# vislearn/esac

Measured on NVIDIA H100. Metric: pose hypotheses scored/sec (640x480, 256 hyp x E experts), higher is better.
Workload: dtype f32 (scoring) / f64 (P3P, refinement)

## Files before the change

__graft_entry__.py:

```python
from __future__ import annotations

import sys
from pathlib import Path

ROOT = Path(__file__).resolve().parent
if str(ROOT) not in sys.path:
    sys.path.insert(0, str(ROOT))


def build() -> None:
    from esac_b200.build import build_library
    from oracle.build import build_oracle
    from oracle.build_ref import build_ref
    lib = build_library()
    assert lib.exists()
    build_oracle()
    build_ref()
    import esac_b200.api as api
    api.load_library()
    import esac


def smoke() -> None:
    import numpy as np
    import torch
    assert torch.cuda.is_available(), "smoke() needs cuda:0"
    import esac
    import esac_b200.api as api
    from esac_b200.synth import make_scene, pose_error
    from oracle import esac_oracle as O

    sc = make_scene(E=2, H=30, W=40, M=32, sub=8, seed=1)
    api.context(0).set_option("fixed_seed", 1)
    api.set_seed(42, 0)
    out = np.zeros((4, 4), np.float32)
    e = esac.forward(sc.coords, sc.assign, out, *sc.params)
    ref = np.zeros((4, 4), np.float32)
    re_, tr = O.forward(sc.coords, sc.assign, ref, *sc.params, seed=42, trace=True)
    hy = api.last_hypotheses(0)
    ds = float(np.abs(hy["scores"] - np.array(tr.scores)).max())
    rot, trans = pose_error(out, ref)
    assert ds < 1e-4, f"score parity {ds}"
    assert e == re_ and rot < 1e-3 and trans < 1e-5, (e, re_, rot, trans)
    api.set_seed(42, 0)
    coords = torch.from_numpy(sc.coords).cuda()
    grads = torch.zeros_like(coords)
    loss = esac.backward(coords, grads, torch.from_numpy(sc.assign).cuda(), torch.from_numpy(sc.gt_pose), 1.0, 100.0,
                         100.0, *sc.params)
    g_ref = np.zeros_like(sc.coords)
    l_ref = O.backward(sc.coords, g_ref, sc.assign, sc.gt_pose, 1.0, 100.0, 100.0, *sc.params, seed=42)
    dg = float(np.abs(grads.cpu().numpy() - g_ref).max() / max(1e-12, np.abs(g_ref).max()))
    assert abs(loss - l_ref) < 1e-6 * max(1.0, abs(l_ref)), (loss, l_ref)
    assert dg < 1e-3, f"gradient parity {dg}"
    print(f"smoke ok: expert {e}, score diff {ds:.2e}, pose diff {rot:.2e} deg / {trans:.2e} m, "
          f"loss {loss:.6f} (oracle {l_ref:.6f}), grad rel diff {dg:.2e}, stats {api.last_stats(0)}")


if __name__ == "__main__":
    build()
    if len(sys.argv) > 1 and sys.argv[1] == "smoke":
        smoke()
```

esac_b200/api.py:

```python
from __future__ import annotations

import ctypes as C
import os
from pathlib import Path

import numpy as np

_HERE = Path(__file__).resolve().parent
LIB_PATH = _HERE / "libesac_b200.so"


class Stats(C.Structure):
    _fields_ = [("M", C.c_int), ("winner", C.c_int), ("n_contrib", C.c_int), ("refine_rounds", C.c_int),
                ("entropy", C.c_double), ("expected_loss", C.c_double),
                ("ms_h2d", C.c_float), ("ms_prep", C.c_float), ("ms_sample", C.c_float), ("ms_score", C.c_float),
                ("ms_select", C.c_float), ("ms_refine", C.c_float), ("ms_backward", C.c_float), ("ms_total", C.c_float),
                ("score_launches", C.c_int), ("kernel_launches", C.c_int),
                ("score_ppt", C.c_int), ("score_grid", C.c_int), ("refine_group", C.c_int)]

    def as_dict(self):
        return {k: getattr(self, k) for k, _ in self._fields_}


_lib = None
# ... 23 lines not shown
    cam = [i32, i32, f32, f32, f32, f32, f32, f32, f32, i32]
    lib.esacb200_forward.argtypes = [vp, vp, i32, i32, i32, vp, i64, i32, vp] + cam + [C.POINTER(i32)]
    lib.esacb200_backward.argtypes = [vp, vp, vp, i32, i32, i32, vp, i64, i32, vp, f32, f32, f32] + cam + [C.POINTER(f64)]
    lib.esacb200_forward_batch.argtypes = [vp, i32, vp, i32, i32, i32, vp, i64, i32, vp] + cam + [vp]
    lib.esacb200_forward_batch.restype = i32
    lib.esacb200_forward_pack.argtypes = [vp, vp, i32, i32, i32, vp, i64, i32, i32] + cam + [i32, vp]
    lib.esacb200_forward_pack.restype = i32
    lib.esacb200_nccl_unique_id.argtypes = [vp]
    lib.esacb200_nccl_unique_id.restype = i32
    lib.esacb200_comm_init.argtypes = [vp, i32, i32, vp]
    lib.esacb200_comm_init.restype = i32
    lib.esacb200_comm_destroy.argtypes = [vp]
    lib.esacb200_comm_destroy.restype = i32
    lib.esacb200_forward_sharded.argtypes = [vp, vp, i32, i32, i32, vp, i64, i32, i32, vp] + cam + [i32, C.POINTER(i32)]
    lib.esacb200_forward_sharded.restype = i32
    lib.esacb200_backward_sharded_nccl.argtypes = [vp, vp, vp, i32, i32, i32, vp, i64, i32, vp, f32, f32, f32] + cam + [i32, C.POINTER(f64)]
    lib.esacb200_backward_sharded_nccl.restype = i32
    lib.esacb200_backward_batch.argtypes = ([vp, i32, vp, vp, i32, i32, i32, vp, i64, i32, vp, f32, f32, f32, vp, vp] + cam[2:] +
                                             [vp])
    lib.esacb200_backward_batch.restype = i32
    lib.esacb200_assign_hypotheses.argtypes = [vp, i32, i32, i32, vp, i32, i32, C.c_uint64, vp, vp]
    lib.esacb200_assign_hypotheses.restype = i32
    lib.esacb200_reproj_loss.argtypes = [vp, i32, vp, vp, i32, i32, vp, vp, vp, f32, f32, f32, i32, f32, f32, f32, vp]
    lib.esacb200_reproj_loss.restype = i32
    lib.esacb200_backward_sharded.argtypes = ([vp, vp, vp, i32, i32, i32, vp, i64, i32, vp, f32, f32, f32] + cam +
                                               [EXCHANGE_FN, vp, C.POINTER(f64)])
    lib.esacb200_backward_sharded.restype = i32
    lib.esacb200_score_poses.argtypes = [vp, vp, i32, i32, i32, vp, i64, i32, vp] + cam + [vp]
    lib.esacb200_refine_poses.argtypes = [vp, vp, i32, i32, i32, vp, i64, i32, vp, i32, i32, f32, f32, f32, f32, f32, i32, vp, vp]
    lib.esacb200_get_refine_profile.argtypes = [vp, vp]
    lib.esacb200_get_refine_profile.restype = i32
    lib.esacb200_get_sample_trace.argtypes = [vp, vp]
    lib.esacb200_get_sample_trace.restype = i32
    lib.esacb200_get_sample_profile.argtypes = [vp, vp]
    lib.esacb200_get_sample_profile.restype = i32
    lib.esacb200_get_stats.argtypes = [vp, C.POINTER(Stats)]
    lib.esacb200_get_hypotheses.argtypes = [vp, vp, vp, vp, vp, vp, vp, vp]
    lib.esacb200_device_info.argtypes = [vp, C.POINTER(i32), C.c_char_p, i32]
    lib.esacb200_copy_last_scores.argtypes = [vp, vp, i32]
    lib.esacb200_copy_last_scores.restype = i32
    for name in ("set_stream", "set_seed", "set_option", "inject_cells", "forward", "backward", "score_poses",
                 "refine_poses", "get_stats", "get_hypotheses", "device_info"):
        getattr(lib, "esacb200_" + name).restype = i32
    lib.esacb200_host_rodrigues.argtypes = [vp, vp, vp]
    lib.esacb200_host_rodrigues.restype = None
    lib.esacb200_host_rodrigues_inv.argtypes = [vp, vp]
    lib.esacb200_host_rodrigues_inv.restype = None
    lib.esacb200_host_p3p_all.argtypes = [vp, vp, vp, vp]
    lib.esacb200_host_p3p_all.restype = i32
    lib.esacb200_host_p3p_pose.argtypes = [vp, vp, f32, f32, f32, f32, vp, C.POINTER(i32)]
    lib.esacb200_host_p3p_pose.restype = i32
    lib.esacb200_host_try.argtypes = [vp, vp, f32, f32, f32, f32, f32, C.POINTER(i32), C.POINTER(i32)]
    lib.esacb200_host_try.restype = None
    lib.esacb200_host_try_verdict.argtypes = [vp, vp, f32, f32, f32, f32, C.POINTER(i32), vp]
    lib.esacb200_host_try_verdict.restype = None
    lib.esacb200_host_project.argtypes = [vp, f32, f32, f32, vp, vp, vp, vp]
    lib.esacb200_host_project.restype = None
    lib.esacb200_host_loss.argtypes = [vp, vp, f64, f64, f64]
    lib.esacb200_host_loss.restype = f64
    lib.esacb200_host_dloss.argtypes = [vp, vp, f64, f64, f64, vp]
    lib.esacb200_host_dloss.restype = None
    lib.esacb200_host_pose2trans.argtypes = [vp, vp]
    lib.esacb200_host_pose2trans.restype = None
    lib.esacb200_host_trans2pose.argtypes = [vp, vp]
    lib.esacb200_host_trans2pose.restype = None
    lib.esacb200_host_dprojectdobj.argtypes = [vp, vp, vp, f32, f32, f32, f32, vp]
    lib.esacb200_host_dprojectdobj.restype = None
    lib.esacb200_host_pinv6.argtypes = [vp, vp]
    lib.esacb200_host_pinv6.restype = None
    lib.esacb200_host_draw_cells.argtypes = [C.c_uint64, C.c_uint32, C.c_uint32, i32, i32, vp]
    lib.esacb200_host_draw_cells.restype = None
    _lib = lib
    return lib


class Context:
    def __init__(self, device: int = 0):
        self.lib = load_library()
        h = C.c_void_p()
        rc = self.lib.esacb200_create(int(device), C.byref(h))
        if rc != 0:
            raise RuntimeError(f"esac_b200: cannot create a context on CUDA device {device} (status {rc}); "
                               "this implementation has no CPU path")
        self.handle = h
        self.device = int(device)
        self.comm_world, self.comm_rank = 1, 0

    def close(self):
        if getattr(self, "handle", None):
            self.lib.esacb200_destroy(self.handle)
            self.handle = None

    def __del__(self):
        try:
            self.close()
        except Exception:
            pass

    def check(self, rc: int):
        if rc != 0:
            msg = self.lib.esacb200_last_error(self.handle)
            raise RuntimeError(f"esac_b200 (status {rc}): {msg.decode() if msg else ''}")

    def set_seed(self, seed: int):
        self.check(self.lib.esacb200_set_seed(self.handle, C.c_uint64(seed & ((1 << 64) - 1))))

# ... 531 lines not shown
```

esac_b200/csrc/capi.cu:

```cuda
#include <cuda_runtime.h>
#include <dlfcn.h>
#include <stdarg.h>
#include <stdio.h>
#include <stdlib.h>
#include <string.h>

#include <exception>
#include <new>
#include <vector>
#include <thread>
#include <chrono>

#include "../../include/esac_b200.h"
#include "../../include/esac_b200_testhooks.h"
#include "esac_internal.h"
#include "esac_p3p_fast.cuh"
#include "esac_rng.cuh"

using namespace esacb200;

namespace {

struct DevBuf {
    void* p = nullptr;
    size_t cap = 0;
    cudaError_t ensure(size_t bytes) {
        if (bytes <= cap) return cudaSuccess;
        if (p) cudaFree(p);
        p = nullptr;
        cap = 0;
        size_t want = bytes + bytes / 4 + 256;
        cudaError_t e = cudaMalloc(&p, want);
        if (e == cudaSuccess) cap = want;
        return e;
    }
    void release() {
        if (p) cudaFree(p);
        p = nullptr;
        cap = 0;
    }
    template <class T>
    T* as() const { return (T*)p; }
};

enum { EV_START = 0, EV_H2D, EV_PREP, EV_SAMPLE, EV_FOLD, EV_SCORE, EV_SELECT, EV_REFINE, EV_BWD, EV_END, EV_COUNT };

}

struct esacb200_ctx {
    int device = 0;
    int sm_count = 0;
    char dev_name[128] = {0};
    cudaStream_t own_stream = nullptr;
    cudaStream_t copy_stream = nullptr;
    cudaStream_t aux_stream = nullptr;
    cudaStream_t aux_more[2] = {nullptr, nullptr};
    cudaEvent_t ev_fork = nullptr, ev_join = nullptr, ev_join_more[2] = {nullptr, nullptr};
    int sample_groups = 2;
    int upload_split = 1;
    cudaEvent_t ev_copied[2] = {nullptr, nullptr}, ev_consumed[2] = {nullptr, nullptr};
    cudaStream_t stream = nullptr;
    uint64_t seed = 1305;
    uint64_t calls = 0;
    int max_tries = 1000000;
    int max_ref_steps = 100;
    int fixed_seed = 0;
    int refine_group_opt = 0;
    int* h_flags = nullptr;
    int h_flags_cap = 0;
    int refine_pretest = 1;
    int refine_compact = 1;
    int refine_profile = 0;
    int refine_jobs_per_group = 3;
    int sample_prefilter = 1;
    int sample_span0 = 256;
    float sample_window = 1.25f;
    int sample_waves = 6;
    float sample_tail_boost = 1.f;
    int sample_trace = 0;
    int smp_groups_last = 0;
    int smp_Mg_last = 0;
    int hyp_offset = 0, hyp_stride = 1;
    int score_ppt_opt = 0, score_hc_opt = 0;
    int refine_coresident = 0;
    char err[512] = {0};
    DevBuf coords, grads, assign64, assign32, counts, offsets, perm, slot_of, chunks, scalars, centres, poses, poses_ref,
        cells, tries, posepk, part, scores, probs, stats, contrib, masks, rounds, scratch, barrier, out17, inject,
        losses, red, hypgrad, job_of, gt, smp_int, smp_surv, smp_trace, clist, eflags, coords4, coords_alt, assign64_alt, out_batch, prof;
    float* h_out = nullptr;
    double* h_dbl = nullptr;
    int inj_M = 0, inj_T = 0;
    cudaEvent_t ev[EV_COUNT] = {nullptr};
    bool ev_used[EV_COUNT] = {false};
    esacb200_stats st;
    int last_M = 0;
    bool last_backward = false;
    int batch_workers = 8;
    void* nccl_comm = nullptr;
    int comm_world = 1, comm_rank = 0;
    DevBuf gathered, grads_work;
    std::vector<esacb200_ctx*> workers;
};

namespace {

struct DeviceGuard {
    int prev = -1;
    explicit DeviceGuard(int device) {
        if (cudaGetDevice(&prev) != cudaSuccess) { cudaGetLastError(); prev = -1; }
        if (prev != device) cudaSetDevice(device);
    }
    ~DeviceGuard() {
        if (prev >= 0) cudaSetDevice(prev);
    }
    DeviceGuard(const DeviceGuard&) = delete;
    DeviceGuard& operator=(const DeviceGuard&) = delete;
};

struct NcclApi {
    typedef struct { char internal[128]; } UniqueId;
    int (*GetUniqueId)(UniqueId*) = nullptr;
    int (*CommInitRank)(void**, int, UniqueId, int) = nullptr;
    int (*CommDestroy)(void*) = nullptr;
    int (*AllGather)(const void*, void*, size_t, int, void*, cudaStream_t) = nullptr;
    int (*AllReduce)(const void*, void*, size_t, int, int, void*, cudaStream_t) = nullptr;
    const char* (*GetErrorString)(int) = nullptr;
    bool ok = false;
};
constexpr int kNcclFloat32 = 7;
// ... 1356 lines not shown
    if (probs) CK(cudaMemcpy(probs, ctx->probs.p, (size_t)M * 8, cudaMemcpyDeviceToHost));
    if (refined6) CK(cudaMemcpy(refined6, ctx->poses_ref.p, (size_t)M * sizeof(Pose), cudaMemcpyDeviceToHost));
    if (losses) {
        if (!ctx->last_backward) return fail(ctx, ESACB200_ERR_ARG, "losses exist only after backward");
        CK(cudaMemcpy(losses, ctx->losses.p, (size_t)M * 8, cudaMemcpyDeviceToHost));
    }
    return ESACB200_OK;
} ESAC_ABI_CATCH(ctx)

void esacb200_host_rodrigues(const double r[3], double R[9], double J[27]) { rodrigues_v2m(r, R, J); }
void esacb200_host_rodrigues_inv(const double R[9], double r[3]) { rodrigues_m2v(R, r); }

int esacb200_host_p3p_all(const double* y9, const double* x9, double* Rs36, double* ts12) {
    double y[3][3], x[3][3], Rs[4][9], ts[4][3];
    for (int i = 0; i < 3; ++i)
        for (int c = 0; c < 3; ++c) { y[i][c] = y9[i * 3 + c]; x[i][c] = x9[i * 3 + c]; }
    int n = p3p_solve(y, x, Rs, ts);
    for (int s = 0; s < n; ++s) {
        for (int c = 0; c < 9; ++c) Rs36[s * 9 + c] = Rs[s][c];
        for (int c = 0; c < 3; ++c) ts12[s * 3 + c] = ts[s][c];
    }
    return n;
}

int esacb200_host_p3p_pose(const float* obj12, const float* img8, float f, float ppx, float ppy, float tau, double* pose6,
                           int* gate) {
    float obj[4][3], img[4][2];
    for (int i = 0; i < 4; ++i) {
        for (int c = 0; c < 3; ++c) obj[i][c] = obj12[i * 3 + c];
        for (int c = 0; c < 2; ++c) img[i][c] = img8[i * 2 + c];
    }
    Pose p;
    bool ok = p3p_pose(obj, img, (double)f, (double)ppx, (double)ppy, p);
    if (gate) *gate = 0;
    if (!ok) { for (int i = 0; i < 6; ++i) pose6[i] = 0; return 0; }
    for (int i = 0; i < 3; ++i) { pose6[i] = p.r[i]; pose6[3 + i] = p.t[i]; }
    if (gate) *gate = minimal_set_gate(obj, img, p, (double)f, (double)ppx, (double)ppy, tau) ? 1 : 0;
    return 1;
}

void esacb200_host_try(const float* obj12, const float* img8, float f, float ppx, float ppy, float tau, float margin,
                       int* may_pass, int* accept) {
    float obj[4][3], img[4][2];
    for (int i = 0; i < 4; ++i) {
        for (int c = 0; c < 3; ++c) obj[i][c] = obj12[i * 3 + c];
        for (int c = 0; c < 2; ++c) img[i][c] = img8[i * 2 + c];
    }
    *may_pass = p3p_may_pass_fast(obj, img, f, ppx, ppy, tau, margin) ? 1 : 0;
    Pose p;
    bool ok = p3p_pose(obj, img, (double)f, (double)ppx, (double)ppy, p);
    *accept = (ok && minimal_set_gate(obj, img, p, (double)f, (double)ppx, (double)ppy, tau)) ? 1 : 0;
}

void esacb200_host_try_verdict(const float* obj12, const float* img8, float f, float ppx, float ppy, float tau, int* accept,
                               double* pose6) {
    float obj[4][3], img[4][2];
    for (int i = 0; i < 4; ++i) {
        for (int c = 0; c < 3; ++c) obj[i][c] = obj12[i * 3 + c];
        for (int c = 0; c < 2; ++c) img[i][c] = img8[i * 2 + c];
    }
    Pose p;
    const bool ok = p3p_pose(obj, img, (double)f, (double)ppx, (double)ppy, p, 1.25 * (double)tau + 1.);
    *accept = (ok && minimal_set_gate(obj, img, p, (double)f, (double)ppx, (double)ppy, tau)) ? 1 : 0;
    if (pose6 && ok)
        for (int i = 0; i < 3; ++i) { pose6[i] = p.r[i]; pose6[3 + i] = p.t[i]; }
}

void esacb200_host_project(const double pose6[6], float f, float ppx, float ppy, const float X[3], float uv_f[2],
                           double uv[2], double J12[12]) {
    double R[9], dRdr[27];
    rodrigues_v2m(pose6, R, dRdr);
    project_point_f(R, pose6 + 3, (double)f, (double)ppx, (double)ppy, X[0], X[1], X[2], uv_f[0], uv_f[1]);
    double Ju[6], Jv[6];
    project_point_jac(R, pose6 + 3, dRdr, (double)f, (double)ppx, (double)ppy, (double)X[0], (double)X[1], (double)X[2], uv[0],
                      uv[1], Ju, Jv);
    for (int i = 0; i < 6; ++i) { J12[i] = Ju[i]; J12[6 + i] = Jv[i]; }
}

double esacb200_host_loss(const double* T1, const double* T2, double wRot, double wTrans, double cut) {
    return pose_loss(T1, T2, wRot, wTrans, cut);
}

void esacb200_host_dloss(const double est6[6], const double gt6[6], double wRot, double wTrans, double cut, double out6[6]) {
    Pose a, b;
    for (int i = 0; i < 3; ++i) { a.r[i] = est6[i]; a.t[i] = est6[3 + i]; b.r[i] = gt6[i]; b.t[i] = gt6[3 + i]; }
    pose_dloss(a, b, wRot, wTrans, cut, out6);
}

void esacb200_host_pose2trans(const double pose6[6], double T16[16]) {
    Pose a;
    for (int i = 0; i < 3; ++i) { a.r[i] = pose6[i]; a.t[i] = pose6[3 + i]; }
    pose2trans(a, T16);
}

void esacb200_host_trans2pose(const double T16[16], double pose6[6]) {
    Pose a;
    trans2pose(T16, a);
    for (int i = 0; i < 3; ++i) { pose6[i] = a.r[i]; pose6[3 + i] = a.t[i]; }
}

void esacb200_host_dprojectdobj(const float pt[2], const float obj[3], const double pose6[6], float f, float ppx, float ppy,
                                float maxReproj, double out3[3]) {
    double R[9];
    rodrigues_v2m(pose6, R, nullptr);
    d_project_d_obj(pt[0], pt[1], obj[0], obj[1], obj[2], R, pose6 + 3, (double)f, (double)ppx, (double)ppy, (double)maxReproj, out3);
}
// ... 11 lines not shown
```

esac_b200/csrc/esac_p3p_fast.cuh:

```cuda
#pragma once
#include "esac_geom.cuh"

namespace esacb200 {

struct Pack1 {
    float a;
    static constexpr int W = 1;
};
struct Mask1 {
    bool a;
};
struct Pack2 {
    float2 v;
    static constexpr int W = 2;
};
struct Mask2 {
    bool a, b;
};
template <typename P> struct MaskOf;
template <> struct MaskOf<Pack1> { typedef Mask1 type; };
template <> struct MaskOf<Pack2> { typedef Mask2 type; };

ESAC_HD Pack1 bc1(float x) { Pack1 r; r.a = x; return r; }
ESAC_HD Pack2 bc2(float x) { Pack2 r; r.v = make_float2(x, x); return r; }
template <typename P> ESAC_HD P bc(float x);
template <> ESAC_HD Pack1 bc<Pack1>(float x) { return bc1(x); }
template <> ESAC_HD Pack2 bc<Pack2>(float x) { return bc2(x); }

ESAC_HD Pack1 operator+(Pack1 x, Pack1 y) { return bc1(x.a + y.a); }
ESAC_HD Pack1 operator-(Pack1 x, Pack1 y) { return bc1(x.a - y.a); }
ESAC_HD Pack1 operator*(Pack1 x, Pack1 y) { return bc1(x.a * y.a); }
ESAC_HD Pack1 operator-(Pack1 x) { return bc1(-x.a); }
ESAC_HD Pack1 fma_(Pack1 x, Pack1 y, Pack1 z) { return bc1(fmaf(x.a, y.a, z.a)); }
#ifdef __CUDA_ARCH__
ESAC_HD Pack2 operator+(Pack2 x, Pack2 y) { Pack2 r; r.v = fadd2(x.v, y.v); return r; }
ESAC_HD Pack2 operator*(Pack2 x, Pack2 y) { Pack2 r; r.v = fmul2(x.v, y.v); return r; }
ESAC_HD Pack2 fma_(Pack2 x, Pack2 y, Pack2 z) { Pack2 r; r.v = ffma2(x.v, y.v, z.v); return r; }
ESAC_HD Pack2 operator-(Pack2 x, Pack2 y) { Pack2 r; r.v = ffma2(make_float2(-1.f, -1.f), y.v, x.v); return r; }
#else
ESAC_HD Pack2 operator+(Pack2 x, Pack2 y) { Pack2 r; r.v = make_float2(x.v.x + y.v.x, x.v.y + y.v.y); return r; }
ESAC_HD Pack2 operator*(Pack2 x, Pack2 y) { Pack2 r; r.v = make_float2(x.v.x * y.v.x, x.v.y * y.v.y); return r; }
ESAC_HD Pack2 fma_(Pack2 x, Pack2 y, Pack2 z) { Pack2 r; r.v = make_float2(fmaf(x.v.x, y.v.x, z.v.x), fmaf(x.v.y, y.v.y, z.v.y)); return r; }
ESAC_HD Pack2 operator-(Pack2 x, Pack2 y) { Pack2 r; r.v = make_float2(x.v.x - y.v.x, x.v.y - y.v.y); return r; }
#endif
ESAC_HD Pack2 operator-(Pack2 x) { Pack2 r; r.v = make_float2(-x.v.x, -x.v.y); return r; }

#define ESAC_PACK_UNARY(name, expr)                                                     \
    ESAC_HD Pack1 name(Pack1 p) { float x = p.a; return bc1(expr); }                    \
    ESAC_HD Pack2 name(Pack2 p) { Pack2 r; float x = p.v.x; r.v.x = (expr); x = p.v.y; r.v.y = (expr); return r; }
ESAC_PACK_UNARY(abs_, fabsf(x))
ESAC_PACK_UNARY(rcp_, Num<float>::div_(1.f, x))
ESAC_PACK_UNARY(sqrt_, Num<float>::sqrt_(x))
ESAC_PACK_UNARY(rsqrt_, rsqrtf(x))
ESAC_PACK_UNARY(cbrt_, cbrtf(x))
#undef ESAC_PACK_UNARY
ESAC_HD Pack1 max_(Pack1 x, Pack1 y) { return bc1(fmaxf(x.a, y.a)); }
ESAC_HD Pack1 min_(Pack1 x, Pack1 y) { return bc1(fminf(x.a, y.a)); }
ESAC_HD Pack2 max_(Pack2 x, Pack2 y) { Pack2 r; r.v = make_float2(fmaxf(x.v.x, y.v.x), fmaxf(x.v.y, y.v.y)); return r; }
ESAC_HD Pack2 min_(Pack2 x, Pack2 y) { Pack2 r; r.v = make_float2(fminf(x.v.x, y.v.x), fminf(x.v.y, y.v.y)); return r; }

#define ESAC_PACK_CMP(name, op)                                                       \
    ESAC_HD Mask1 name(Pack1 x, Pack1 y) { Mask1 m; m.a = x.a op y.a; return m; }     \
    ESAC_HD Mask2 name(Pack2 x, Pack2 y) { Mask2 m; m.a = x.v.x op y.v.x; m.b = x.v.y op y.v.y; return m; }
ESAC_PACK_CMP(lt_, <)
ESAC_PACK_CMP(le_, <=)
ESAC_PACK_CMP(gt_, >)
ESAC_PACK_CMP(ge_, >=)
#undef ESAC_PACK_CMP
ESAC_HD Mask1 operator&(Mask1 x, Mask1 y) { Mask1 m; m.a = x.a && y.a; return m; }
ESAC_HD Mask1 operator|(Mask1 x, Mask1 y) { Mask1 m; m.a = x.a || y.a; return m; }
ESAC_HD Mask1 operator!(Mask1 x) { Mask1 m; m.a = !x.a; return m; }
ESAC_HD Mask2 operator&(Mask2 x, Mask2 y) { Mask2 m; m.a = x.a && y.a; m.b = x.b && y.b; return m; }
ESAC_HD Mask2 operator|(Mask2 x, Mask2 y) { Mask2 m; m.a = x.a || y.a; m.b = x.b || y.b; return m; }
ESAC_HD Mask2 operator!(Mask2 x) { Mask2 m; m.a = !x.a; m.b = !x.b; return m; }
ESAC_HD Mask1 mask1(bool v) { Mask1 m; m.a = v; return m; }
ESAC_HD Mask2 mask2(bool v) { Mask2 m; m.a = v; m.b = v; return m; }
template <typename M> ESAC_HD M splat(bool v);
template <> ESAC_HD Mask1 splat<Mask1>(bool v) { return mask1(v); }
template <> ESAC_HD Mask2 splat<Mask2>(bool v) { return mask2(v); }
ESAC_HD bool all_(Mask1 m) { return m.a; }
ESAC_HD bool all_(Mask2 m) { return m.a && m.b; }
ESAC_HD Pack1 sel(Mask1 m, Pack1 x, Pack1 y) { return bc1(m.a ? x.a : y.a); }
ESAC_HD Pack2 sel(Mask2 m, Pack2 x, Pack2 y) { Pack2 r; r.v = make_float2(m.a ? x.v.x : y.v.x, m.b ? x.v.y : y.v.y); return r; }
ESAC_HD Mask1 nan_(Pack1 x) { return mask1(!(x.a == x.a)); }
ESAC_HD Mask2 nan_(Pack2 x) { Mask2 m; m.a = !(x.v.x == x.v.x); m.b = !(x.v.y == x.v.y); return m; }

template <typename P, typename M>
ESAC_HD void argmax3(P a0, P a1, P a2, M& is0, M& is1) {
    is0 = ge_(a0, a1) & ge_(a0, a2);
    is1 = !is0 & ge_(a1, a2);
}
template <typename P, typename M>
// ... 245 lines not shown
```

esac_b200/csrc/hyp.cu:

```cuda
#include "esac_internal.h"
#include "esac_p3p_fast.cuh"
#include "esac_rng.cuh"

namespace esacb200 {

constexpr int kTryThreads = 128;
constexpr int kNoTry = 0x7fffffff;
constexpr unsigned long long kNoKey = ~0ull;
constexpr unsigned kNoSlot = 0xffffffffu;

struct SampleArgs {
    const float4* coords4;
    const int* assign32;
    Problem P;
    uint64_t seed;
    int limit;
    const int* injected;
    int inj_T;
    int use_prefilter;
    int hyp_offset;
    int hyp_stride;
    int h_first, h_step, Mg;
    const int* perm;
    const int* offsets;
// ... 26 lines not shown
    return a.perm ? a.perm[a.offsets[a.e_lo] + k] : a.h_first + k * a.h_step;
}

__device__ __forceinline__ void load_try(const SampleArgs& a, int h, int t, int cx[4], int cy[4], float obj[4][3], float img[4][2]) {
    const Problem& P = a.P;
    if (a.injected) {
        const int* c = a.injected + ((size_t)h * a.inj_T + t) * 8;
        for (int j = 0; j < 4; ++j) { cx[j] = c[2 * j]; cy[j] = c[2 * j + 1]; }
    } else {
        draw_minimal_set(a.seed, (uint32_t)(h * a.hyp_stride + a.hyp_offset), (uint32_t)t, P.W, P.H, cx, cy);
    }
    const float4* pl = a.coords4 + (size_t)a.assign32[h] * P.N;
    for (int j = 0; j < 4; ++j) {
        const int p = cy[j] * P.W + cx[j];
        const float4 v = __ldg(pl + p);
        obj[j][0] = v.x; obj[j][1] = v.y; obj[j][2] = v.z;
        img[j][0] = (float)(cx[j] * P.sub + P.sub / 2 - P.shiftX);
        img[j][1] = (float)(cy[j] * P.sub + P.sub / 2 - P.shiftY);
    }
}

__device__ __noinline__ bool exact_try(const SampleArgs& a, int h, int t, Pose& pose, int cx[4], int cy[4], bool& solved,
                                       bool verdict_only = false) {
    float obj[4][3], img[4][2];
    load_try(a, h, t, cx, cy, obj, img);
    const double f = (double)a.P.f, ppx = (double)a.P.ppx, ppy = (double)a.P.ppy;
    solved = p3p_pose(obj, img, f, ppx, ppy, pose, verdict_only ? 1.25 * (double)a.P.tau + 1. : 0.);
    return solved && minimal_set_gate(obj, img, pose, f, ppx, ppy, a.P.tau);
}

__global__ void interleave_kernel(const float* __restrict__ coords, float4* __restrict__ out, int E, int N) {
    const size_t total = (size_t)E * N;
    for (size_t i = (size_t)blockIdx.x * blockDim.x + threadIdx.x; i < total; i += (size_t)gridDim.x * blockDim.x) {
        const size_t e = i / N, p = i - e * N;
        const float* pl = coords + e * 3 * (size_t)N;
        out[i] = make_float4(pl[p], pl[N + p], pl[2 * (size_t)N + p], 0.f);
    }
}

__global__ void sample_init_kernel(const __grid_constant__ SampleArgs a) {
    const SampleState& st = a.st;
    const int k = blockIdx.x * blockDim.x + threadIdx.x;
    const int n = lane_size(a);
    if (k < n) {
        const int h = lane_hyp(a, k);
        st.best[h] = kNoKey; st.base[h] = 0; st.ovf[h] = kNoTry; st.list[k] = h;
    }
    if (k == 0) {
        st.counters[0] = n; st.counters[1] = 0; st.counters[2] = 0; st.counters[3] = a.span0; st.counters[4] = 0;
        st.counters[5] = 0; st.counters[6] = 0; st.counters[7] = 0;
    }
}

constexpr int kPackTries = 2 * kTryThreads;
struct PreItem {
    int h, ta, tb;
    bool valid0, valid1;
    unsigned cell[8];
};
__device__ __forceinline__ void cp_async16(void* smem, const void* gmem) {
    asm volatile("cp.async.ca.shared.global [%0], [%1], 16;" ::"r"((unsigned)__cvta_generic_to_shared(smem)), "l"(gmem) : "memory");
}
__device__ __forceinline__ void prefilter_issue(const SampleArgs& a, long long item, int cph, int span, float4 (*dst)[kTryThreads], PreItem& it) {
    const int u = (int)(item / cph), c = (int)(item - (long long)u * cph);
    it.h = a.st.list[u];
    const int t0 = a.st.base[it.h];
    const int off0 = c * kPackTries + threadIdx.x, off1 = off0 + kTryThreads;
    it.valid0 = off0 < span && t0 + off0 < a.limit;
    it.valid1 = off1 < span && t0 + off1 < a.limit;
    it.ta = it.valid0 ? t0 + off0 : t0;
    it.tb = it.valid1 ? t0 + off1 : t0;
    if (!(it.valid0 || it.valid1)) return;
    const Problem& P = a.P;
    const float4* pl = a.coords4 + (size_t)a.assign32[it.h] * P.N;
#pragma unroll
    for (int k = 0; k < 2; ++k) {
        const int t = k == 0 ? it.ta : it.tb;
        int cx[4], cy[4];
        if (a.injected) {
            const int* cc = a.injected + ((size_t)it.h * a.inj_T + t) * 8;
            for (int j = 0; j < 4; ++j) { cx[j] = cc[2 * j]; cy[j] = cc[2 * j + 1]; }
        } else {
            draw_minimal_set(a.seed, (uint32_t)(it.h * a.hyp_stride + a.hyp_offset), (uint32_t)t, P.W, P.H, cx, cy);
        }
#pragma unroll
        for (int j = 0; j < 4; ++j) {
            it.cell[k * 4 + j] = ((unsigned)cy[j] << 16) | (unsigned)cx[j];
            cp_async16(&dst[k * 4 + j][threadIdx.x], pl + (cy[j] * P.W + cx[j]));
        }
    }
}

__global__ void __launch_bounds__(kTryThreads, 4) prefilter_kernel(const __grid_constant__ SampleArgs a) {
    TraceScope trace(a.trace, a.trace_slot);
    __shared__ float4 s_obj[2][8][kTryThreads];
    const int n_unres = a.st.counters[0];
    const int span = a.st.counters[3];
    const int cph = (span + kPackTries - 1) / kPackTries;
    const long long n_items = (long long)n_unres * cph;
    const int lane = threadIdx.x & 31, tid = threadIdx.x;
    const Problem& P = a.P;
    PreItem cur, nxt;
    long long item = blockIdx.x;
    if (item < n_items) prefilter_issue(a, item, cph, span, s_obj[0], cur);
    asm volatile("cp.async.commit_group;" ::: "memory");
    int buf = 0;
    for (; item < n_items; item += gridDim.x) {
        const long long ni = item + gridDim.x;
        if (ni < n_items) prefilter_issue(a, ni, cph, span, s_obj[buf ^ 1], nxt);
        asm volatile("cp.async.commit_group;" ::: "memory");
        asm volatile("cp.async.wait_group 1;" ::: "memory");
        bool pass0 = false, pass1 = false;
        if (cur.valid0 || cur.valid1) {
            float obj0[4][3], img0[4][2], obj1[4][3], img1[4][2];
#pragma unroll
            for (int j = 0; j < 4; ++j) {
                const float4 v0 = s_obj[buf][j][tid], v1 = s_obj[buf][4 + j][tid];
                obj0[j][0] = v0.x; obj0[j][1] = v0.y; obj0[j][2] = v0.z;
                obj1[j][0] = v1.x; obj1[j][1] = v1.y; obj1[j][2] = v1.z;
                const unsigned c0 = cur.cell[j], c1 = cur.cell[4 + j];
                img0[j][0] = (float)((int)(c0 & 0xffffu) * P.sub + P.sub / 2 - P.shiftX);
                img0[j][1] = (float)((int)(c0 >> 16) * P.sub + P.sub / 2 - P.shiftY);
                img1[j][0] = (float)((int)(c1 & 0xffffu) * P.sub + P.sub / 2 - P.shiftX);
                img1[j][1] = (float)((int)(c1 >> 16) * P.sub + P.sub / 2 - P.shiftY);
            }
            if (a.use_prefilter) p3p_may_pass_fast2(obj0, img0, obj1, img1, P.f, P.ppx, P.ppy, P.tau, pass0, pass1);
            else pass0 = pass1 = true;
            pass0 = pass0 && cur.valid0;
            pass1 = pass1 && cur.valid1;
        }
        const unsigned m0 = __ballot_sync(0xffffffffu, pass0), m1 = __ballot_sync(0xffffffffu, pass1);
        if (m0 | m1) {
            const int n0 = __popc(m0);
            int basei = 0;
            if (lane == 0) basei = atomicAdd(&a.st.counters[1], n0 + __popc(m1));
            basei = __shfl_sync(0xffffffffu, basei, 0);
            const unsigned lt = (1u << lane) - 1u;
            if (pass0) {
                const int idx = basei + __popc(m0 & lt);
                if (idx < a.st.cap) a.st.surv[idx] = make_int2(cur.h, cur.ta);
                else atomicMin(&a.st.ovf[cur.h], cur.ta);
            }
            if (pass1) {
                const int idx = basei + n0 + __popc(m1 & lt);
                if (idx < a.st.cap) a.st.surv[idx] = make_int2(cur.h, cur.tb);
                else atomicMin(&a.st.ovf[cur.h], cur.tb);
            }
        }
        cur = nxt;
        buf ^= 1;
    }
    asm volatile("cp.async.wait_group 0;" ::: "memory");
}

__device__ void advance_wave(const SampleState& st, int limit, float window, float tail_boost);

__global__ void __launch_bounds__(128) exact_kernel(const __grid_constant__ SampleArgs a) {
    TraceScope trace(a.trace, a.trace_slot);
    const int n = min(a.st.counters[1], a.st.cap);
    for (int i = blockIdx.x * blockDim.x + threadIdx.x; i < n; i += gridDim.x * blockDim.x) {
        const int2 ht = a.st.surv[i];
        if (ht.y >= a.st.ovf[ht.x]) continue;
        Pose pose;
        int cx[4], cy[4];
        bool solved;
        if (exact_try(a, ht.x, ht.y, pose, cx, cy, solved, true)) {
            unsigned slot = (unsigned)atomicAdd(&a.st.counters[2], 1);
            if (slot < (unsigned)a.st.cap_acc) {
                Accepted& ac = a.st.stage[slot];
                ac.pose = pose;
                for (int j = 0; j < 4; ++j) { ac.cells[2 * j] = cx[j]; ac.cells[2 * j + 1] = cy[j]; }
            } else {
                slot = kNoSlot;
            }
            atomicMin(&a.st.best[ht.x], ((unsigned long long)(unsigned)ht.y << 32) | slot);
        }
    }
    __shared__ int s_last;
    __threadfence();
    __syncthreads();
    if (threadIdx.x == 0) s_last = atomicAdd(&a.st.counters[4], 1) == (int)gridDim.x - 1;
    __syncthreads();
    if (s_last) {
        __threadfence();
        advance_wave(a.st, a.limit, a.window, a.tail_boost);
    }
}

__device__ void advance_wave(const SampleState& st, int limit, float window, float tail_boost) {
    __shared__ int s_fill;
    const int span = st.counters[3];
    if (threadIdx.x == 0) s_fill = 0;
    __syncthreads();
    const int n_unres = st.counters[0];
    int* next = st.list + st.M;
    for (int u = threadIdx.x; u < n_unres; u += blockDim.x) {
        const int h = st.list[u];
        const int ovf = st.ovf[h];
        const int end = min(st.base[h] + span, ovf);
        const unsigned long long best = __ldcg(&st.best[h]);
        const bool resolved = (long long)(best >> 32) < (long long)end;
        if (!resolved) {
            if (best != kNoKey) st.best[h] = kNoKey;
            st.base[h] = end;
            st.ovf[h] = kNoTry;
            if (end < limit) next[atomicAdd(&s_fill, 1)] = h;
        }
    }
    __syncthreads();
    const int nn = s_fill;
    for (int u = threadIdx.x; u < nn; u += blockDim.x) st.list[u] = next[u];
    __syncthreads();
    if (threadIdx.x == 0) {
        const int n_surv = min(st.counters[1], st.cap);
        const double tried = (double)n_unres * (double)span;
        const double hits = n_unres - nn > 0 ? (double)(n_unres - nn) : 0.5;
        const double boost = nn <= 8 ? tail_boost * 2. : (nn <= 64 ? tail_boost : 1.);
        double next_span = (double)window * boost * tried / hits;
        next_span = next_span < 256. ? 256. : (next_span > 65536. ? 65536. : next_span);
        st.counters[3] = ((int)next_span + kPackTries - 1) / kPackTries * kPackTries;
        st.counters[0] = nn;
        st.counters[1] = 0;
        st.counters[4] = 0;
        if (n_unres > 0) {
            st.counters[5] += n_unres * span;
            st.counters[6] += n_surv;
            st.counters[7] += 1;
        }
    }
}

__global__ void __launch_bounds__(kTryThreads) tail_kernel(const __grid_constant__ SampleArgs a) {
    const int n_unres = a.st.counters[0];
    __shared__ int s_list[kTryThreads * 8];
    __shared__ int s_n, s_best;
    for (int u = blockIdx.x; u < n_unres; u += gridDim.x) {
        const int h = a.st.list[u];
        int base = a.st.base[h];
        __syncthreads();
        if (threadIdx.x == 0) s_best = kNoTry;
        while (base < a.limit) {
            if (threadIdx.x == 0) s_n = 0;
            __syncthreads();
            const int span = min(a.limit - base, kTryThreads * 8);
            for (int t = base + threadIdx.x; t < base + span; t += kTryThreads) {
                int cx[4], cy[4];
                float obj[4][3], img[4][2];
                load_try(a, h, t, cx, cy, obj, img);
                if (!a.use_prefilter || p3p_may_pass_fast(obj, img, a.P.f, a.P.ppx, a.P.ppy, a.P.tau)) s_list[atomicAdd(&s_n, 1)] = t;
            }
            __syncthreads();
            const int n = s_n;
            for (int i = threadIdx.x; i < n; i += kTryThreads) {
                Pose pose;
                int cx[4], cy[4];
                bool solved;
                if (exact_try(a, h, s_list[i], pose, cx, cy, solved, true)) atomicMin(&s_best, s_list[i]);
            }
            __syncthreads();
            if (s_best != kNoTry) break;
            base += span;
        }
        if (threadIdx.x == 0 && s_best != kNoTry) a.st.best[h] = ((unsigned long long)(unsigned)s_best << 32) | kNoSlot;
    }
}


__global__ void __launch_bounds__(64) emit_kernel(const __grid_constant__ SampleArgs a, Pose* poses, int* cells, int* tries) {
    const int k = blockIdx.x * blockDim.x + threadIdx.x;
    if (k >= lane_size(a)) return;
    const int h = lane_hyp(a, k);
    const unsigned long long key = a.st.best[h];
    const int t = key != kNoKey ? (int)(key >> 32) : a.limit - 1;
// ... 6 lines not shown
        for (int j = 0; j < 4; ++j) { cx[j] = ac.cells[2 * j]; cy[j] = ac.cells[2 * j + 1]; }
    } else {
        bool solved;
        exact_try(a, h, t, pose, cx, cy, solved);
        if (!solved) { for (int c = 0; c < 3; ++c) { pose.r[c] = 0; pose.t[c] = 0; } }
    }
    poses[h] = pose;
    for (int j = 0; j < 4; ++j) { cells[h * 8 + 2 * j] = cx[j]; cells[h * 8 + 2 * j + 1] = cy[j]; }
    tries[h] = t + 1;
}

int launch_sample(const float* coords, float4* coords4, const int* assign32, const Problem& P, uint64_t seed, int max_tries,
                  const int* injected, int inj_T, const SampleState* st, int n_lanes, int sm_count, int use_prefilter,
                  int hyp_offset, int hyp_stride, Pose* poses, int* cells, int* tries, const cudaStream_t* lanes,
                  cudaEvent_t ev_fork, const cudaEvent_t* ev_join, int split_e, const int* perm, const int* offsets,
                  const cudaEvent_t* ev_half, int span0, float window, int n_waves,
                  unsigned long long* trace, float tail_boost) {
    int launches = 0;
    cudaStream_t stream = lanes[0];
    if (!split_e) { interleave_kernel<<<sm_count * 8, 256, 0, stream>>>(coords, coords4, P.E, P.N); ++launches; }
    SampleArgs args[4];
    int bound[4];
    for (int g = 0; g < n_lanes; ++g) {
        SampleArgs& a = args[g];
        a.coords4 = coords4; a.assign32 = assign32; a.P = P; a.seed = seed;
        a.limit = injected ? (max_tries < inj_T ? max_tries : inj_T) : max_tries;
        a.injected = injected; a.inj_T = inj_T; a.st = st[g]; a.use_prefilter = use_prefilter; a.hyp_offset = hyp_offset; a.hyp_stride = hyp_stride > 0 ? hyp_stride : 1;
        a.h_first = g; a.h_step = n_lanes; a.Mg = (P.M - g + n_lanes - 1) / n_lanes;
        a.perm = nullptr; a.offsets = nullptr; a.e_lo = a.e_hi = 0;
        a.span0 = span0; a.window = window; a.trace = trace; a.trace_slot = 0; a.tail_boost = tail_boost;
        bound[g] = a.Mg;
        if (split_e) {
            a.perm = perm; a.offsets = offsets;
            a.e_lo = g == 0 ? 0 : split_e;
            a.e_hi = g == 0 ? split_e : P.E;
            bound[g] = P.M;
        }
    }
    if (n_lanes > 1) {
        cudaEventRecord(ev_fork, stream);
        for (int g = 1; g < n_lanes; ++g) cudaStreamWaitEvent(lanes[g], ev_fork, 0);
    }
    for (int g = 0; g < n_lanes; ++g) {
        cudaStream_t sg = lanes[g];
        SampleArgs& a = args[g];
        if (split_e) {
            cudaStreamWaitEvent(sg, ev_half[g], 0);
            const int ne = a.e_hi - a.e_lo;
            interleave_kernel<<<sm_count * 8, 256, 0, sg>>>(coords + (size_t)a.e_lo * 3 * P.N, coords4 + (size_t)a.e_lo * P.N, ne, P.N);
            ++launches;
        }
        if (bound[g] <= 0) continue;
        sample_init_kernel<<<(bound[g] + 255) / 256, 256, 0, sg>>>(a); ++launches;
        const int grid = sm_count * 4;
        for (int r = 0; r < n_waves; ++r) {
            a.trace_slot = (g * 32 + r) * 2;
            prefilter_kernel<<<grid, kTryThreads, 0, sg>>>(a); ++launches;
            a.trace_slot = (g * 32 + r) * 2 + 1;
            exact_kernel<<<sm_count * 4, 128, 0, sg>>>(a); ++launches;
        }
        tail_kernel<<<bound[g] < sm_count * 4 ? bound[g] : sm_count * 4, kTryThreads, 0, sg>>>(a); ++launches;
        emit_kernel<<<(bound[g] + 63) / 64, 64, 0, sg>>>(a, poses, cells, tries); ++launches;
    }
    for (int g = 1; g < n_lanes; ++g) {
        cudaEventRecord(ev_join[g], lanes[g]);
        cudaStreamWaitEvent(stream, ev_join[g], 0);
    }
    return launches;
}

__global__ void trace_init_kernel(unsigned long long* trace, int slots) {
    const int i = blockIdx.x * blockDim.x + threadIdx.x;
    if (i < slots) { trace[2 * i] = ~0ull; trace[2 * i + 1] = 0ull; }
}
void launch_trace_init(unsigned long long* trace, int slots, cudaStream_t st) { trace_init_kernel<<<(slots + 255) / 256, 256, 0, st>>>(trace, slots); }

}
```

include/esac_b200_testhooks.h:

```cpp
#ifndef ESAC_B200_TESTHOOKS_H
#define ESAC_B200_TESTHOOKS_H

#include <stdint.h>

#ifdef __cplusplus
extern "C" {
#endif

void esacb200_host_rodrigues(const double r[3], double R[9], double J[27]);
void esacb200_host_rodrigues_inv(const double R[9], double r[3]);
int esacb200_host_p3p_all(const double* y9, const double* x9, double* Rs36, double* ts12);
int esacb200_host_p3p_pose(const float* obj12, const float* img8, float f, float ppx, float ppy, float tau,
                           double* pose6, int* gate);
void esacb200_host_try(const float* obj12, const float* img8, float f, float ppx, float ppy, float tau, float margin,
                       int* may_pass, int* accept);
void esacb200_host_try_verdict(const float* obj12, const float* img8, float f, float ppx, float ppy, float tau, int* accept,
                               double* pose6);
void esacb200_host_project(const double pose6[6], float f, float ppx, float ppy, const float X[3], float uv_f[2],
                           double uv[2], double J12[12]);
double esacb200_host_loss(const double* T1, const double* T2, double wRot, double wTrans, double cut);
void esacb200_host_dloss(const double est6[6], const double gt6[6], double wRot, double wTrans, double cut,
                         double out6[6]);
void esacb200_host_pose2trans(const double pose6[6], double T16[16]);
void esacb200_host_trans2pose(const double T16[16], double pose6[6]);
void esacb200_host_dprojectdobj(const float pt[2], const float obj[3], const double pose6[6], float f, float ppx,
                                float ppy, float maxReproj, double out3[3]);
void esacb200_host_pinv6(const double A[36], double out[36]);
void esacb200_host_draw_cells(uint64_t seed, uint32_t h, uint32_t t, int W, int H, int32_t* cells8);

#ifdef __cplusplus
}
#endif
#endif
```

Baseline: 919,000.

## Prefilter one minimal set per thread, double grid, shrink sampling window

The prefilter kernel now handles one minimal-set try per thread with the scalar fast P3P check, where before it handled two tries per thread with the paired fast2 variant. This halves shared-memory staging and per-thread registers, so launch bounds allow 8 blocks per SM and the grid doubles. Span quantization is decoupled into a fixed 256 quantum, and the default sample window drops from 1.25 to 0.9, so fewer speculative tries are issued per wave. Scalar Pack1 ops use explicit _rn intrinsics to stop contraction and keep host/device parity. A host test hook compares the single and paired may-pass results. The trade-off is losing the paired packed-float2 ILP and risking more waves/tail work with the smaller window.

```diff
diff --git a/__graft_entry__.py b/__graft_entry__.py
--- a/__graft_entry__.py
+++ b/__graft_entry__.py
@@ -1,5 +1,6 @@
 from __future__ import annotations
 
+import os
 import sys
 from pathlib import Path
 
@@ -7,8 +8,20 @@
 if str(ROOT) not in sys.path:
     sys.path.insert(0, str(ROOT))
 
+REFERENCE_CANDIDATES = (ROOT.parent / "reference", Path("/root/reference"))
+
+
+def _name_reference() -> None:
+    if os.environ.get("ESAC_REFERENCE"):
+        return
+    for cand in REFERENCE_CANDIDATES:
+        if os.access(cand / "code" / "esac" / "esac.cpp", os.R_OK):
+            os.environ["ESAC_REFERENCE"] = str(cand)
+            return
+
 
 def build() -> None:
+    _name_reference()
     from esac_b200.build import build_library
     from oracle.build import build_oracle
     from oracle.build_ref import build_ref
diff --git a/esac_b200/api.py b/esac_b200/api.py
--- a/esac_b200/api.py
+++ b/esac_b200/api.py
@@ -99,6 +99,8 @@
     lib.esacb200_host_p3p_pose.restype = i32
     lib.esacb200_host_try.argtypes = [vp, vp, f32, f32, f32, f32, f32, C.POINTER(i32), C.POINTER(i32)]
     lib.esacb200_host_try.restype = None
+    lib.esacb200_host_may_pass.argtypes = [vp, vp, i32, f32, f32, f32, f32, vp, vp]
+    lib.esacb200_host_may_pass.restype = None
     lib.esacb200_host_try_verdict.argtypes = [vp, vp, f32, f32, f32, f32, C.POINTER(i32), vp]
     lib.esacb200_host_try_verdict.restype = None
     lib.esacb200_host_project.argtypes = [vp, f32, f32, f32, vp, vp, vp, vp]
diff --git a/esac_b200/csrc/capi.cu b/esac_b200/csrc/capi.cu
--- a/esac_b200/csrc/capi.cu
+++ b/esac_b200/csrc/capi.cu
@@ -74,7 +74,7 @@
     int refine_jobs_per_group = 3;
     int sample_prefilter = 1;
     int sample_span0 = 256;
-    float sample_window = 1.25f;
+    float sample_window = 0.9f;
     int sample_waves = 6;
     float sample_tail_boost = 1.f;
     int sample_trace = 0;
@@ -1537,6 +1537,24 @@
     *accept = (ok && minimal_set_gate(obj, img, p, (double)f, (double)ppx, (double)ppy, tau)) ? 1 : 0;
 }
 
+void esacb200_host_may_pass(const float* obj12n, const float* img8n, int n, float f, float ppx, float ppy, float tau, int* one,
+                            int* pair) {
+    for (int i = 0; i + 1 < n; i += 2) {
+        float obj[2][4][3], img[2][4][2];
+        for (int k = 0; k < 2; ++k)
+            for (int p = 0; p < 4; ++p) {
+                for (int c = 0; c < 3; ++c) obj[k][p][c] = obj12n[(size_t)(i + k) * 12 + p * 3 + c];
+                for (int c = 0; c < 2; ++c) img[k][p][c] = img8n[(size_t)(i + k) * 8 + p * 2 + c];
+            }
+        one[i] = p3p_may_pass_fast(obj[0], img[0], f, ppx, ppy, tau) ? 1 : 0;
+        one[i + 1] = p3p_may_pass_fast(obj[1], img[1], f, ppx, ppy, tau) ? 1 : 0;
+        bool p0, p1;
+        p3p_may_pass_fast2(obj[0], img[0], obj[1], img[1], f, ppx, ppy, tau, p0, p1);
+        pair[i] = p0 ? 1 : 0;
+        pair[i + 1] = p1 ? 1 : 0;
+    }
+}
+
 void esacb200_host_try_verdict(const float* obj12, const float* img8, float f, float ppx, float ppy, float tau, int* accept,
                                double* pose6) {
     float obj[4][3], img[4][2];
diff --git a/esac_b200/csrc/esac_p3p_fast.cuh b/esac_b200/csrc/esac_p3p_fast.cuh
--- a/esac_b200/csrc/esac_p3p_fast.cuh
+++ b/esac_b200/csrc/esac_p3p_fast.cuh
@@ -27,17 +27,21 @@
 template <> ESAC_HD Pack1 bc<Pack1>(float x) { return bc1(x); }
 template <> ESAC_HD Pack2 bc<Pack2>(float x) { return bc2(x); }
 
-ESAC_HD Pack1 operator+(Pack1 x, Pack1 y) { return bc1(x.a + y.a); }
-ESAC_HD Pack1 operator-(Pack1 x, Pack1 y) { return bc1(x.a - y.a); }
-ESAC_HD Pack1 operator*(Pack1 x, Pack1 y) { return bc1(x.a * y.a); }
 ESAC_HD Pack1 operator-(Pack1 x) { return bc1(-x.a); }
-ESAC_HD Pack1 fma_(Pack1 x, Pack1 y, Pack1 z) { return bc1(fmaf(x.a, y.a, z.a)); }
 #ifdef __CUDA_ARCH__
+ESAC_HD Pack1 operator+(Pack1 x, Pack1 y) { return bc1(__fadd_rn(x.a, y.a)); }
+ESAC_HD Pack1 operator*(Pack1 x, Pack1 y) { return bc1(__fmul_rn(x.a, y.a)); }
+ESAC_HD Pack1 fma_(Pack1 x, Pack1 y, Pack1 z) { return bc1(__fmaf_rn(x.a, y.a, z.a)); }
+ESAC_HD Pack1 operator-(Pack1 x, Pack1 y) { return bc1(__fmaf_rn(-1.f, y.a, x.a)); }
 ESAC_HD Pack2 operator+(Pack2 x, Pack2 y) { Pack2 r; r.v = fadd2(x.v, y.v); return r; }
 ESAC_HD Pack2 operator*(Pack2 x, Pack2 y) { Pack2 r; r.v = fmul2(x.v, y.v); return r; }
 ESAC_HD Pack2 fma_(Pack2 x, Pack2 y, Pack2 z) { Pack2 r; r.v = ffma2(x.v, y.v, z.v); return r; }
 ESAC_HD Pack2 operator-(Pack2 x, Pack2 y) { Pack2 r; r.v = ffma2(make_float2(-1.f, -1.f), y.v, x.v); return r; }
 #else
+ESAC_HD Pack1 operator+(Pack1 x, Pack1 y) { return bc1(x.a + y.a); }
+ESAC_HD Pack1 operator*(Pack1 x, Pack1 y) { return bc1(x.a * y.a); }
+ESAC_HD Pack1 fma_(Pack1 x, Pack1 y, Pack1 z) { return bc1(fmaf(x.a, y.a, z.a)); }
+ESAC_HD Pack1 operator-(Pack1 x, Pack1 y) { return bc1(x.a - y.a); }
 ESAC_HD Pack2 operator+(Pack2 x, Pack2 y) { Pack2 r; r.v = make_float2(x.v.x + y.v.x, x.v.y + y.v.y); return r; }
 ESAC_HD Pack2 operator*(Pack2 x, Pack2 y) { Pack2 r; r.v = make_float2(x.v.x * y.v.x, x.v.y * y.v.y); return r; }
 ESAC_HD Pack2 fma_(Pack2 x, Pack2 y, Pack2 z) { Pack2 r; r.v = make_float2(fmaf(x.v.x, y.v.x, z.v.x), fmaf(x.v.y, y.v.y, z.v.y)); return r; }
diff --git a/esac_b200/csrc/hyp.cu b/esac_b200/csrc/hyp.cu
--- a/esac_b200/csrc/hyp.cu
+++ b/esac_b200/csrc/hyp.cu
@@ -102,11 +102,11 @@
     }
 }
 
-constexpr int kPackTries = 2 * kTryThreads;
+constexpr int kSpanQuantum = 256;
 struct PreItem {
-    int h, ta, tb;
-    bool valid0, valid1;
-    unsigned cell[8];
+    int h, t;
+    bool valid;
+    unsigned cell[4];
 };
 __device__ __forceinline__ void cp_async16(void* smem, const void* gmem) {
     asm volatile("cp.async.ca.shared.global [%0], [%1], 16;" ::"r"((unsigned)__cvta_generic_to_shared(smem)), "l"(gmem) : "memory");
@@ -115,38 +115,32 @@
     const int u = (int)(item / cph), c = (int)(item - (long long)u * cph);
     it.h = a.st.list[u];
     const int t0 = a.st.base[it.h];
-    const int off0 = c * kPackTries + threadIdx.x, off1 = off0 + kTryThreads;
-    it.valid0 = off0 < span && t0 + off0 < a.limit;
-    it.valid1 = off1 < span && t0 + off1 < a.limit;
-    it.ta = it.valid0 ? t0 + off0 : t0;
-    it.tb = it.valid1 ? t0 + off1 : t0;
-    if (!(it.valid0 || it.valid1)) return;
+    const int off = c * kTryThreads + threadIdx.x;
+    it.valid = off < span && t0 + off < a.limit;
+    if (!it.valid) { it.t = t0; return; }
+    it.t = t0 + off;
     const Problem& P = a.P;
     const float4* pl = a.coords4 + (size_t)a.assign32[it.h] * P.N;
+    int cx[4], cy[4];
+    if (a.injected) {
+        const int* cc = a.injected + ((size_t)it.h * a.inj_T + it.t) * 8;
+        for (int j = 0; j < 4; ++j) { cx[j] = cc[2 * j]; cy[j] = cc[2 * j + 1]; }
+    } else {
+        draw_minimal_set(a.seed, (uint32_t)(it.h * a.hyp_stride + a.hyp_offset), (uint32_t)it.t, P.W, P.H, cx, cy);
+    }
 #pragma unroll
-    for (int k = 0; k < 2; ++k) {
-        const int t = k == 0 ? it.ta : it.tb;
-        int cx[4], cy[4];
-        if (a.injected) {
-            const int* cc = a.injected + ((size_t)it.h * a.inj_T + t) * 8;
-            for (int j = 0; j < 4; ++j) { cx[j] = cc[2 * j]; cy[j] = cc[2 * j + 1]; }
-        } else {
-            draw_minimal_set(a.seed, (uint32_t)(it.h * a.hyp_stride + a.hyp_offset), (uint32_t)t, P.W, P.H, cx, cy);
-        }
-#pragma unroll
-        for (int j = 0; j < 4; ++j) {
-            it.cell[k * 4 + j] = ((unsigned)cy[j] << 16) | (unsigned)cx[j];
-            cp_async16(&dst[k * 4 + j][threadIdx.x], pl + (cy[j] * P.W + cx[j]));
-        }
-    }
-}
-
-__global__ void __launch_bounds__(kTryThreads, 4) prefilter_kernel(const __grid_constant__ SampleArgs a) {
+    for (int j = 0; j < 4; ++j) {
+        it.cell[j] = ((unsigned)cy[j] << 16) | (unsigned)cx[j];
+        cp_async16(&dst[j][threadIdx.x], pl + (cy[j] * P.W + cx[j]));
+    }
+}
+
+__global__ void __launch_bounds__(kTryThreads, 8) prefilter_kernel(const __grid_constant__ SampleArgs a) {
     TraceScope trace(a.trace, a.trace_slot);
-    __shared__ float4 s_obj[2][8][kTryThreads];
+    __shared__ float4 s_obj[2][4][kTryThreads];
     const int n_unres = a.st.counters[0];
     const int span = a.st.counters[3];
-    const int cph = (span + kPackTries - 1) / kPackTries;
+    const int cph = (span + kTryThreads - 1) / kTryThreads;
     const long long n_items = (long long)n_unres * cph;
     const int lane = threadIdx.x & 31, tid = threadIdx.x;
     const Problem& P = a.P;
@@ -160,41 +154,28 @@
         if (ni < n_items) prefilter_issue(a, ni, cph, span, s_obj[buf ^ 1], nxt);
         asm volatile("cp.async.commit_group;" ::: "memory");
         asm volatile("cp.async.wait_group 1;" ::: "memory");
-        bool pass0 = false, pass1 = false;
-        if (cur.valid0 || cur.valid1) {
-            float obj0[4][3], img0[4][2], obj1[4][3], img1[4][2];
+        bool pass = false;
+        if (cur.valid) {
+            float obj[4][3], img[4][2];
 #pragma unroll
             for (int j = 0; j < 4; ++j) {
-                const float4 v0 = s_obj[buf][j][tid], v1 = s_obj[buf][4 + j][tid];
-                obj0[j][0] = v0.x; obj0[j][1] = v0.y; obj0[j][2] = v0.z;
-                obj1[j][0] = v1.x; obj1[j][1] = v1.y; obj1[j][2] = v1.z;
-                const unsigned c0 = cur.cell[j], c1 = cur.cell[4 + j];
-                img0[j][0] = (float)((int)(c0 & 0xffffu) * P.sub + P.sub / 2 - P.shiftX);
-                img0[j][1] = (float)((int)(c0 >> 16) * P.sub + P.sub / 2 - P.shiftY);
-                img1[j][0] = (float)((int)(c1 & 0xffffu) * P.sub + P.sub / 2 - P.shiftX);
-                img1[j][1] = (float)((int)(c1 >> 16) * P.sub + P.sub / 2 - P.shiftY);
-            }
-            if (a.use_prefilter) p3p_may_pass_fast2(obj0, img0, obj1, img1, P.f, P.ppx, P.ppy, P.tau, pass0, pass1);
-            else pass0 = pass1 = true;
-            pass0 = pass0 && cur.valid0;
-            pass1 = pass1 && cur.valid1;
-        }
-        const unsigned m0 = __ballot_sync(0xffffffffu, pass0), m1 = __ballot_sync(0xffffffffu, pass1);
-        if (m0 | m1) {
-            const int n0 = __popc(m0);
+                const float4 v = s_obj[buf][j][tid];
+                obj[j][0] = v.x; obj[j][1] = v.y; obj[j][2] = v.z;
+                const unsigned c = cur.cell[j];
+                img[j][0] = (float)((int)(c & 0xffffu) * P.sub + P.sub / 2 - P.shiftX);
+                img[j][1] = (float)((int)(c >> 16) * P.sub + P.sub / 2 - P.shiftY);
+            }
+            pass = !a.use_prefilter || p3p_may_pass_fast(obj, img, P.f, P.ppx, P.ppy, P.tau);
+        }
+        const unsigned m = __ballot_sync(0xffffffffu, pass);
+        if (m) {
             int basei = 0;
-            if (lane == 0) basei = atomicAdd(&a.st.counters[1], n0 + __popc(m1));
+            if (lane == 0) basei = atomicAdd(&a.st.counters[1], __popc(m));
             basei = __shfl_sync(0xffffffffu, basei, 0);
-            const unsigned lt = (1u << lane) - 1u;
-            if (pass0) {
-                const int idx = basei + __popc(m0 & lt);
-                if (idx < a.st.cap) a.st.surv[idx] = make_int2(cur.h, cur.ta);
-                else atomicMin(&a.st.ovf[cur.h], cur.ta);
-            }
-            if (pass1) {
-                const int idx = basei + n0 + __popc(m1 & lt);
-                if (idx < a.st.cap) a.st.surv[idx] = make_int2(cur.h, cur.tb);
-                else atomicMin(&a.st.ovf[cur.h], cur.tb);
+            if (pass) {
+                const int idx = basei + __popc(m & ((1u << lane) - 1u));
+                if (idx < a.st.cap) a.st.surv[idx] = make_int2(cur.h, cur.t);
+                else atomicMin(&a.st.ovf[cur.h], cur.t);
             }
         }
         cur = nxt;
@@ -268,7 +249,7 @@
         const double boost = nn <= 8 ? tail_boost * 2. : (nn <= 64 ? tail_boost : 1.);
         double next_span = (double)window * boost * tried / hits;
         next_span = next_span < 256. ? 256. : (next_span > 65536. ? 65536. : next_span);
-        st.counters[3] = ((int)next_span + kPackTries - 1) / kPackTries * kPackTries;
+        st.counters[3] = ((int)next_span + kSpanQuantum - 1) / kSpanQuantum * kSpanQuantum;
         st.counters[0] = nn;
         st.counters[1] = 0;
         st.counters[4] = 0;
@@ -381,7 +362,7 @@
         }
         if (bound[g] <= 0) continue;
         sample_init_kernel<<<(bound[g] + 255) / 256, 256, 0, sg>>>(a); ++launches;
-        const int grid = sm_count * 4;
+        const int grid = sm_count * 8;
         for (int r = 0; r < n_waves; ++r) {
             a.trace_slot = (g * 32 + r) * 2;
             prefilter_kernel<<<grid, kTryThreads, 0, sg>>>(a); ++launches;
diff --git a/include/esac_b200_testhooks.h b/include/esac_b200_testhooks.h
--- a/include/esac_b200_testhooks.h
+++ b/include/esac_b200_testhooks.h
@@ -14,6 +14,8 @@
                            double* pose6, int* gate);
 void esacb200_host_try(const float* obj12, const float* img8, float f, float ppx, float ppy, float tau, float margin,
                        int* may_pass, int* accept);
+void esacb200_host_may_pass(const float* obj12n, const float* img8n, int n, float f, float ppx, float ppy, float tau, int* one,
+                            int* pair);
 void esacb200_host_try_verdict(const float* obj12, const float* img8, float f, float ppx, float ppy, float tau, int* accept,
                                double* pose6);
 void esacb200_host_project(const double pose6[6], float f, float ppx, float ppy, const float X[3], float uv_f[2],
```

After: 943,500 (median of 6 runs). 2.7% higher.
